# serenedb/serenedb

Measured on NVIDIA H100. Metric: filter->GROUP BY throughput (BASELINE.json configs[1]; bm25 object = configs[2]), higher is better.
Workload: dtype int64+f64

## Files before the change

### serenedb_b200/csrc/column_kernels.cuh

```cuda
#pragma once

#include "device_common.cuh"

namespace sdbg {

constexpr int kMaxPreds = 4;

struct ColDev {
  const void* values;
  const uint64_t* validity;
  int32_t type;
  int32_t pad;
};
struct PredDev {
  ColDev col;
  int32_t op;
  int32_t pad;
  int64_t lo_i, hi_i;
  double lo_f, hi_f;
};
struct PredSet {
  PredDev p[kMaxPreds];
  int32_t n;
  int32_t pad;
// ... 290 lines not shown
  GroupSlot* table;
  unsigned long long* out_of_range;
  const uint8_t* skip;
  const ForBlockDev* hdr[kMaxStreams];
  int32_t pred_stream[kMaxPreds];
  int32_t key_stream, sum_i_stream;
};
constexpr uint32_t kZoneRows = 2048;

__host__ __device__ __forceinline__ long long fkey(long long bits) { return bits ^ ((bits >> 63) & 0x7FFFFFFFFFFFFFFFll); }

__device__ __forceinline__ void fix_limbs(double w, int limb, int eunit, long long& l0, long long& l1) {
  const long long bits = __double_as_longlong(w);
  const int ex = int((bits >> 52) & 0x7FF);
  unsigned long long mant = static_cast<unsigned long long>(bits) & 0xFFFFFFFFFFFFFull;
  if (ex) mant |= 1ull << 52;
  const int s = (ex ? ex : 1) - 1075 - eunit;
  unsigned long long lo, hi = 0ull;
  if (s >= 0) { lo = mant << s; if (s) hi = mant >> (64 - s); }
  else lo = s > -64 ? mant >> (-s) : 0ull;
  l0 = static_cast<long long>(lo & ((1ull << limb) - 1ull));
  l1 = static_cast<long long>((lo >> limb) | (hi << (64 - limb)));
  if (bits < 0) { l0 = -l0; l1 = -l1; }
}
__host__ __device__ __forceinline__ double fix_total(long long s0, long long s1, int limb, int eunit) {
  long long hi = s1 >> (64 - limb);
  unsigned long long lo = static_cast<unsigned long long>(s1) << limb;
  const unsigned long long lo2 = lo + static_cast<unsigned long long>(s0);
  hi += (s0 >> 63) + (lo2 < lo ? 1 : 0);
  lo = lo2;
  const bool neg = hi < 0;
  if (neg) { lo = ~lo + 1ull; hi = ~hi + (lo == 0ull ? 1 : 0); }
  const double mag = static_cast<double>(static_cast<unsigned long long>(hi)) * 18446744073709551616.0 + static_cast<double>(lo);
  return scalbn(neg ? -mag : mag, eunit);
}

template <int kType>
__device__ __forceinline__ void load2(const unsigned char* col, uint32_t r, long long (&v)[2]) {
  if (kType == 2) {
    const int2 x = *reinterpret_cast<const int2*>(col + size_t(r) * 4u);
    v[0] = x.x; v[1] = x.y;
  } else {
    const longlong2 x = *reinterpret_cast<const longlong2*>(col + size_t(r) * 8u);
    v[0] = x.x; v[1] = x.y;
  }
}
template <int kType>
__device__ __forceinline__ uint32_t range2(const unsigned char* col, uint32_t r, long long lo, unsigned long long span) {
  long long v[2];
  load2<kType>(col, r, v);
  if (kType == 1) { v[0] = fkey(v[0]); v[1] = fkey(v[1]); }
  return (static_cast<unsigned long long>(v[0] - lo) <= span ? 1u : 0u) | (static_cast<unsigned long long>(v[1] - lo) <= span ? 2u : 0u);
}
__device__ __forceinline__ void unpack2(const unsigned char* col, uint32_t r, const uint4 h, long long (&v)[2]) {
  const unsigned long long* w = reinterpret_cast<const unsigned long long*>(col);
  const uint32_t bits = h.z;
  const long long base = static_cast<long long>((static_cast<unsigned long long>(h.y) << 32) | h.x);
  const unsigned long long mask = bits >= 64u ? ~0ull : (1ull << bits) - 1ull;
#pragma unroll
  for (int j = 0; j < 2; ++j) {
    const uint32_t bit = (r + uint32_t(j)) * bits, wi = bit >> 6, sh = bit & 63u;
    unsigned long long x = w[wi] >> sh;
    if (sh + bits > 64u) x |= w[wi + 1] << (64u - sh);
    v[j] = base + static_cast<long long>(x & mask);
  }
}
__device__ __forceinline__ uint32_t range2_for(const unsigned char* col, uint32_t r, const uint4 h, long long lo, unsigned long long span) {
  long long v[2];
  unpack2(col, r, h, v);
  return (static_cast<unsigned long long>(v[0] - lo) <= span ? 1u : 0u) | (static_cast<unsigned long long>(v[1] - lo) <= span ? 2u : 0u);
}

template <int kStages, int kTileRows, int kConsumerWarps, bool kPacked, bool kQuad, bool kFor = false>
__global__ void __launch_bounds__((kConsumerWarps + 1) * 32)
filter_groupby_tma_kernel(const TmaGroupByParams P) {
  extern __shared__ __align__(128) unsigned char smem[];
  __shared__ __align__(8) uint64_t full_bar[kStages], empty_bar[kStages];
  static_assert(!kFor || (kForGroupRows % kTileRows == 0 && kTileRows % 128 == 0), "a tile's packed slice must be 16-byte aligned");

  const uint32_t tid = threadIdx.x, warp = tid >> 5, lane = tid & 31u;
  if (tid == 0) {
    for (int s = 0; s < kStages; ++s) { mbar_init(&full_bar[s], 1u); mbar_init(&empty_bar[s], kConsumerWarps); }
    asm volatile("fence.mbarrier_init.release.cluster;" ::: "memory");
  }
  __syncthreads();
  const uint32_t stage_bytes = P.off[P.n_streams];
  const uint64_t n_tiles = (P.rows + kTileRows - 1) / kTileRows;
  uint4* const pk_hdr = reinterpret_cast<uint4*>(smem + size_t(kStages) * stage_bytes + (kQuad ? size_t(kConsumerWarps) * (2048u + 256u) : 0u));

  if (warp == kConsumerWarps) {
    if (kFor) {
      const bool mine = lane < uint32_t(P.n_streams);
      const ForBlockDev* hp = mine ? P.hdr[lane] : nullptr;
      const char* src = mine ? static_cast<const char*>(P.src[lane]) : nullptr;
      const uint32_t elem = mine ? uint32_t(P.elem[lane]) : 0u, soff = mine ? P.off[lane] : 0u;
      auto header = [&](uint64_t t) { return __ldg(reinterpret_cast<const uint4*>(hp + (t * kTileRows) / kForGroupRows)); };
      uint4 nh = make_uint4(0u, 0u, 0u, 0u);
      uint64_t nh_tile = ~0ull;
      uint32_t it = 0;
      for (uint64_t tile = blockIdx.x; tile < n_tiles; tile += gridDim.x) {
        if (P.skip != nullptr && P.skip[(tile * kTileRows) / kZoneRows]) continue;
        uint4 h = make_uint4(0u, 0u, 0u, 0u);
        if (hp != nullptr) h = nh_tile == tile ? nh : header(tile);
        const uint64_t next = tile + gridDim.x;
        if (hp != nullptr && next < n_tiles && (P.skip == nullptr || !P.skip[(next * kTileRows) / kZoneRows])) { nh = header(next); nh_tile = next; }
        const uint32_t st = it % kStages, use = it / kStages;
        ++it;
        const uint64_t row0 = tile * kTileRows;
        const uint32_t nrows = uint32_t(min(static_cast<unsigned long long>(kTileRows), static_cast<unsigned long long>(P.rows - row0)));
        uint32_t bytes = 0u;
        const char* g = nullptr;
        if (hp != nullptr) {
          bytes = (nrows * h.z + 127u) / 128u * 16u;
          g = src + uint64_t(h.w) * 8u + (row0 % kForGroupRows) * h.z / 8u;
        } else if (mine) {
          bytes = (nrows * elem + 15u) & ~15u;
          g = src + row0 * elem;
        }
        const uint32_t total = __reduce_add_sync(kFull, bytes);
        if (lane == 0) mbar_wait(&empty_bar[st], (use & 1u) ^ 1u);
        for (int s = 0; s < P.n_streams; ++s) {
          uint4 x;
          x.x = __shfl_sync(kFull, h.x, s); x.y = __shfl_sync(kFull, h.y, s); x.z = __shfl_sync(kFull, h.z, s); x.w = __shfl_sync(kFull, h.w, s);
          if (lane == 0) pk_hdr[st * kMaxStreams + s] = x;
        }
        if (lane == 0) mbar_arrive_expect_tx(&full_bar[st], total);
        __syncwarp();
        if (bytes != 0u) bulk_g2s(smem + size_t(st) * stage_bytes + soff, g, bytes, &full_bar[st]);
      }
      return;
    }
    if (lane == 0) {
      uint32_t it = 0;
      for (uint64_t tile = blockIdx.x; tile < n_tiles; tile += gridDim.x) {
        if (P.skip != nullptr && P.skip[(tile * kTileRows) / kZoneRows]) continue;
        const uint32_t st = it % kStages, use = it / kStages;
        ++it;
        mbar_wait(&empty_bar[st], (use & 1u) ^ 1u);
        const uint64_t row0 = tile * kTileRows;
        const uint32_t nrows = uint32_t(min(static_cast<unsigned long long>(kTileRows), static_cast<unsigned long long>(P.rows - row0)));
        uint32_t total = 0;
        for (int s = 0; s < P.n_streams; ++s) total += (nrows * uint32_t(P.elem[s]) + 15u) & ~15u;
        mbar_arrive_expect_tx(&full_bar[st], total);
        unsigned char* dst = smem + size_t(st) * stage_bytes;
        for (int s = 0; s < P.n_streams; ++s) {
          const uint32_t bytes = (nrows * uint32_t(P.elem[s]) + 15u) & ~15u;
          bulk_g2s(dst + P.off[s], static_cast<const char*>(P.src[s]) + row0 * uint64_t(P.elem[s]), bytes, &full_bar[st]);
        }
      }
    }
    return;
  }

  unsigned long long* const q_words = reinterpret_cast<unsigned long long*>(smem + size_t(kStages) * stage_bytes) + size_t(warp) * 256u;
  uint32_t* const q_idx = reinterpret_cast<uint32_t*>(smem + size_t(kStages) * stage_bytes + size_t(kConsumerWarps) * 2048u) + size_t(warp) * 64u;
  uint32_t it = 0;
  for (uint64_t tile = blockIdx.x; tile < n_tiles; tile += gridDim.x) {
    if (P.skip != nullptr && P.skip[(tile * kTileRows) / kZoneRows]) continue;
    const uint32_t st = it % kStages, use = it / kStages;
    ++it;
    mbar_wait(&full_bar[st], use & 1u);
    const unsigned char* base = smem + size_t(st) * stage_bytes;
    const uint64_t row0 = tile * kTileRows;
    const uint32_t nrows = uint32_t(min(static_cast<unsigned long long>(kTileRows), static_cast<unsigned long long>(P.rows - row0)));
    const uint32_t pack_word = kPacked ? uint32_t(tile % uint64_t(P.pack_tables)) : 0u;
    const uint4* const hst = pk_hdr + st * kMaxStreams;
    for (uint32_t rb = warp * 64u; rb < nrows; rb += kConsumerWarps * 64u) {
      const uint32_t r = rb + 2u * lane;
      uint32_t m = r + 1u < nrows ? 3u : r < nrows ? 1u : 0u;
#pragma unroll
      for (int i = 0; i < kMaxPreds; ++i) {
        if (i < P.n_preds) {
          const unsigned char* col = base + P.pred_off[i];
          uint32_t in;
          if (kFor && P.pred_type[i] == kTypeFor) in = range2_for(col, r, hst[P.pred_stream[i]], P.pred_lo[i], P.pred_span[i]);
          else switch (P.pred_type[i]) {
            case 0: in = range2<0>(col, r, P.pred_lo[i], P.pred_span[i]); break;
            case 1: in = range2<1>(col, r, P.pred_lo[i], P.pred_span[i]); break;
            default: in = range2<2>(col, r, P.pred_lo[i], P.pred_span[i]); break;
          }
          m &= P.pred_negate[i] ? ~in : in;
        }
      }
      if (!kQuad && m == 0u) continue;
      long long key[2], v[2] = {0, 0};
      double w[2] = {0.0, 0.0};
      if (kFor && P.key_type == kTypeFor) unpack2(base + P.key_off, r, hst[P.key_stream], key);
      else if (P.key_type == 2) load2<2>(base + P.key_off, r, key); else load2<0>(base + P.key_off, r, key);
      if (kPacked || P.has_sum_i) {
        if (kFor && P.sum_i_type == kTypeFor) unpack2(base + P.sum_i_off, r, hst[P.sum_i_stream], v);
        else if (P.sum_i_type == 2) load2<2>(base + P.sum_i_off, r, v); else load2<0>(base + P.sum_i_off, r, v);
      }
      if (P.has_sum_f) {
        const double2 x = *reinterpret_cast<const double2*>(base + P.sum_f_off + size_t(r) * 8u);
        w[0] = x.x; w[1] = x.y;
      }
      if (kQuad) {
        unsigned long long a[2][4];
        uint32_t gi[2] = {0u, 0u};
#pragma unroll
        for (int j = 0; j < 2; ++j) {
          if (!(m & (1u << j))) continue;
          const unsigned long long idx = static_cast<unsigned long long>(key[j] - P.key_min);
          if (idx >= P.key_span) { atomicAdd(P.out_of_range, 1ull); m &= ~(1u << j); continue; }
          gi[j] = uint32_t(idx);
          if (kPacked) {
            const unsigned long long pk = (1ull << P.pack_shift) + static_cast<unsigned long long>(v[j] - P.pack_bias);
            a[j][0] = pack_word == 0u ? pk : 0ull;
            a[j][1] = pack_word == 1u ? pk : 0ull;
            a[j][2] = pack_word == 2u ? pk : 0ull;
          } else {
            a[j][0] = 1ull;
            a[j][1] = !P.has_sum_i ? 0ull : P.wide_int ? (static_cast<unsigned long long>(v[j]) & 0xFFFFFFFFull) : static_cast<unsigned long long>(v[j]);
            a[j][2] = P.has_sum_i && P.wide_int ? static_cast<unsigned long long>(v[j] >> 32) : 0ull;
          }
          a[j][3] = 0ull;
          if (P.fix_limb) {
            long long l0, l1;
// ... 249 lines not shown
      case 1: static_cast<long long*>(out)[i] = static_cast<long long>(h % 1000000ull); break;
      case 2: static_cast<double*>(out)[i] = static_cast<double>(h >> 11) * 0x1.0p-53; break;
      case 3: static_cast<long long*>(out)[i] = static_cast<long long>(h % 2001ull) - 1000ll; break;
      case 4: static_cast<double*>(out)[i] = static_cast<double>(h >> 11) * 0x1.0p-53 * 1000.0; break;
      case 6: static_cast<int*>(out)[i] = static_cast<int>(h % 1000000ull); break;
      case 7: static_cast<long long*>(out)[i] = static_cast<long long>((row0 + i) / 100ull); break;
      default: static_cast<long long*>(out)[i] = static_cast<long long>(h); break;
    }
  }
}

template <typename T>
__global__ void __launch_bounds__(256)
gather_rows_kernel(const T* __restrict__ values, const unsigned long long* __restrict__ validity, const uint32_t* __restrict__ docs,
                   uint64_t n, uint64_t rows, T* __restrict__ out, unsigned char* __restrict__ out_valid) {
  for (uint64_t i = uint64_t(blockIdx.x) * blockDim.x + threadIdx.x; i < n; i += uint64_t(gridDim.x) * blockDim.x) {
    const uint64_t r = uint64_t(docs[i]) - 1ull;
    const bool inside = r < rows;
    const bool ok = inside && (validity == nullptr || ((validity[r >> 6] >> (r & 63ull)) & 1ull));
    out[i] = ok ? values[r] : T(0);
    if (out_valid != nullptr) out_valid[i] = ok ? 1u : 0u;
  }
}

__device__ __forceinline__ long long for_value(const ForBlockDev& h, const unsigned long long* w, uint32_t i) {
  unsigned long long v = 0ull;
  if (h.bits != 0u) {
    const unsigned long long mask = h.bits >= 64u ? ~0ull : ((1ull << h.bits) - 1ull);
    const uint64_t bit = uint64_t(i) * h.bits;
    const uint32_t sh = uint32_t(bit & 63ull);
    const unsigned long long lo = w[bit >> 6] >> sh;
    const unsigned long long hi = (sh != 0u && sh + h.bits > 64u) ? (w[(bit >> 6) + 1ull] << (64u - sh)) : 0ull;
    v = (lo | hi) & mask;
  }
  return h.base + static_cast<long long>(v);
}

__global__ void __launch_bounds__(256)
for_unpack_kernel(const ForBlockDev* __restrict__ headers, const unsigned long long* __restrict__ words, uint64_t rows,
                  long long* __restrict__ out) {
  const uint64_t n_groups = (rows + kForGroupRows - 1) / kForGroupRows;
  const uint32_t lane = threadIdx.x & 31u;
  for (uint64_t g = (uint64_t(blockIdx.x) * blockDim.x + threadIdx.x) >> 5; g < n_groups; g += (uint64_t(gridDim.x) * blockDim.x) >> 5) {
    const ForBlockDev h = headers[g];
    const uint64_t row0 = g * kForGroupRows;
    const uint32_t n = (rows - row0 < kForGroupRows) ? uint32_t(rows - row0) : kForGroupRows;
    for (uint32_t i = lane; i < n; i += 32u) out[row0 + i] = for_value(h, words + h.off8, i);
  }
}

__global__ void __launch_bounds__(256)
for_stats_kernel(const long long* __restrict__ values, const ForBlockDev* __restrict__ packed_hdr,
                 const unsigned long long* __restrict__ words, uint64_t rows, long long* __restrict__ zone,
                 ForBlockDev* __restrict__ hdr, unsigned long long* __restrict__ n_words) {
  const uint64_t n_groups = (rows + kForGroupRows - 1) / kForGroupRows;
  const uint32_t lane = threadIdx.x & 31u;
  for (uint64_t g = (uint64_t(blockIdx.x) * blockDim.x + threadIdx.x) >> 5; g < n_groups; g += (uint64_t(gridDim.x) * blockDim.x) >> 5) {
    const uint64_t row0 = g * kForGroupRows;
    const uint32_t n = (rows - row0 < kForGroupRows) ? uint32_t(rows - row0) : kForGroupRows;
    long long mn = 0x7FFFFFFFFFFFFFFFll, mx = -0x7FFFFFFFFFFFFFFFll - 1;
    for (uint32_t i = lane; i < n; i += 32u) {
      const long long v = words ? for_value(packed_hdr[g], words + packed_hdr[g].off8, i) : values[row0 + i];
      mn = min(mn, v); mx = max(mx, v);
    }
#pragma unroll
    for (int o = 16; o > 0; o >>= 1) { mn = min(mn, __shfl_xor_sync(kFull, mn, o)); mx = max(mx, __shfl_xor_sync(kFull, mx, o)); }
    if (lane == 0) {
      zone[2 * g] = mn; zone[2 * g + 1] = mx;
      if (!words) {
        const unsigned long long span = static_cast<unsigned long long>(mx) - static_cast<unsigned long long>(mn);
        const uint32_t bits = span == 0ull ? 0u : uint32_t(64 - __clzll(static_cast<long long>(span)));
        ForBlockDev h; h.base = mn; h.bits = bits; h.off8 = 0u;
        hdr[g] = h;
        n_words[g] = (uint64_t(n) * bits + 63u) / 64u;
      }
    }
  }
}

__global__ void __launch_bounds__(256)
for_pack_kernel(const long long* __restrict__ values, const ForBlockDev* __restrict__ stats_hdr,
                const unsigned long long* __restrict__ offsets, uint64_t rows, ForBlockDev* __restrict__ hdr,
                unsigned long long* __restrict__ words) {
  const uint64_t n_groups = (rows + kForGroupRows - 1) / kForGroupRows;
  const uint32_t lane = threadIdx.x & 31u;
  for (uint64_t g = (uint64_t(blockIdx.x) * blockDim.x + threadIdx.x) >> 5; g < n_groups; g += (uint64_t(gridDim.x) * blockDim.x) >> 5) {
    ForBlockDev h = stats_hdr[g];
    h.off8 = uint32_t(offsets[g]);
    const uint64_t row0 = g * kForGroupRows;
    const uint32_t n = (rows - row0 < kForGroupRows) ? uint32_t(rows - row0) : kForGroupRows;
    if (lane == 0) hdr[g] = h;
    const uint32_t nw = uint32_t(offsets[g + 1] - offsets[g]);
    for (uint32_t wi = lane; wi < nw; wi += 32u) {
      const uint64_t b0 = uint64_t(wi) * 64u;
      const uint32_t i0 = uint32_t(b0 / h.bits), i1 = min(n - 1u, uint32_t((b0 + 63u) / h.bits));
      unsigned long long word = 0ull;
      for (uint32_t i = i0; i <= i1; ++i) {
        const unsigned long long d = static_cast<unsigned long long>(values[row0 + i]) - static_cast<unsigned long long>(h.base);
        const uint64_t p = uint64_t(i) * h.bits;
        word |= p >= b0 ? d << (p - b0) : d >> (b0 - p);
      }
      words[h.off8 + wi] = word;
    }
    if (g + 1 == n_groups && lane == 0) words[offsets[n_groups]] = 0ull;
  }
}

}
```

### serenedb_b200/csrc/sdbg_abi.cu

```cuda
#include <cuda_runtime.h>
#include <cub/device/device_radix_sort.cuh>
#include <cub/device/device_scan.cuh>
#include <dlfcn.h>
#include <nccl.h>

#include <algorithm>
#include <array>
#include <atomic>
#include <cfloat>
#include <cmath>
#include <cstdio>
#include <cstdlib>
#include <cstring>
#include <map>
#include <memory>
#include <string>
#include <limits>
#include <thread>
#include <vector>

#include "../../include/sdbg.h"
#include "bm25_kernels.cuh"
#include "bm25_stream.cuh"
#include "bm25_merge.cuh"
#include "bm25_count.cuh"
#include "bm25_sort.cuh"
#include "column_kernels.cuh"
#include "posting_format.hpp"

using namespace sdbg;

namespace {

struct DevBuf {
  void* p = nullptr;
  size_t cap = 0;
};

struct ColumnObj {
  void* d_values = nullptr;
  void* d_packed = nullptr;
  size_t packed_bytes = 0;
  uint64_t* d_validity = nullptr;
  int type = 0;
  uint64_t rows = 0;
  bool owned = true;
  bool has_minmax = false;
  int64_t mn = 0, mx = 0;
  long long* d_zone = nullptr;
  bool zone_ok = false;
  bool has_absmax = false;
  uint64_t absmax_bits = 0;
};

}

struct sdbg_ctx {
  int device = 0;
  int sm_count = 132;
  cudaStream_t stream = nullptr;
  cudaStream_t stream2 = nullptr;
  cudaEvent_t ev_fork = nullptr, ev_join = nullptr;
  cudaEvent_t ev0 = nullptr, ev1 = nullptr;
  std::string err;
  uint64_t launches = 0;
  DevBuf scratch[16];
  DevBuf pass[4];
  DevBuf stage_raw;
  void* h_pinned = nullptr;
  size_t h_pinned_cap = 0;
  void* flush = nullptr;
  size_t flush_bytes = 0;
  cudaEvent_t ev_copy[16] = {};
  bool topk_attr_set = false;
  void* nccl_comm = nullptr;
  unsigned long long* h_oor = nullptr;
  void* h_result = nullptr;
  void* d_result = nullptr;
  unsigned long long result_seq = 0;
  size_t h_result_cap = 0;
  bool counter_zeroed = false;
  bool oor_pending = false;
  bool fix_over_pending = false;
  uint64_t zone_blocks_total = 0;
  unsigned long long* d_zone_skipped = nullptr;
  int dist_rank = 0, dist_world = 1;
  int wand = 1;
  bool profiling = false;
  struct ProfSpan { int id; cudaEvent_t a, b; };
  std::vector<ProfSpan> spans;
  std::vector<cudaEvent_t> event_pool;
};

struct sdbg_segment {
  sdbg_ctx* ctx = nullptr;
// ... 356 lines not shown
  CU(c, cudaMalloc(&s->d_norms, rows * width + 16));
  CU(c, cudaMemcpyAsync(s->d_norms, src, rows * width, cudaMemcpyHostToDevice, c->stream));
  CU(c, cudaStreamSynchronize(c->stream));
  s->norm_width = width;
  s->wand_avg_dl = nonzero ? float(double(sum) / double(nonzero)) : 0.f;
  return SDBG_OK;
}

namespace {
size_t type_width(int t) { return t == SDBG_I32 ? 4 : 8; }

uint64_t for_groups(uint64_t rows) { return (rows + kForGroupRows - 1) / kForGroupRows; }
size_t for_hdr_bytes(uint64_t rows) { return (for_groups(rows) * sizeof(ForBlockDev) + 255) & ~size_t(255); }
const ForBlockDev* for_headers(const ColumnObj& col) { return static_cast<const ForBlockDev*>(col.d_packed); }
const unsigned long long* for_words(const ColumnObj& col) {
  return reinterpret_cast<const unsigned long long*>(static_cast<const char*>(col.d_packed) + for_hdr_bytes(col.rows));
}
unsigned grid_per_group_warp(sdbg_ctx* c, uint64_t n_groups) {
  return unsigned(std::max<uint64_t>(1, std::min<uint64_t>((n_groups * 32 + 255) / 256, uint64_t(c->sm_count) * 16)));
}
int ensure_zone(sdbg_ctx* c, ColumnObj& col) {
  if (!col.d_zone) CU(c, cudaMalloc(reinterpret_cast<void**>(&col.d_zone), for_groups(col.rows) * 16));
  return SDBG_OK;
}

int raw_values(sdbg_ctx* c, ColumnObj& col, void** out) {
  if (!col.d_values && col.d_packed) {
    CU(c, cudaMalloc(&col.d_values, col.rows * 8 + 64));
    CU(c, cudaMemsetAsync(static_cast<char*>(col.d_values) + col.rows * 8, 0, 64, c->stream));
    for_unpack_kernel<<<grid_per_group_warp(c, for_groups(col.rows)), 256, 0, c->stream>>>(for_headers(col), for_words(col), col.rows,
                                                                                           static_cast<long long*>(col.d_values));
    ++c->launches;
    CU(c, cudaGetLastError());
  }
  *out = col.d_values;
  return SDBG_OK;
}

int pack_column(sdbg_ctx* c, ColumnObj& col) {
  const uint64_t rows = col.rows, n_groups = for_groups(rows);
  int rc;
  auto keep_raw = [&]() -> int {
    if (col.d_packed) { cudaFree(col.d_packed); col.d_packed = nullptr; col.packed_bytes = 0; }
    CU(c, cudaMalloc(&col.d_values, rows * 8 + 64));
    CU(c, cudaMemcpyAsync(col.d_values, c->stage_raw.p, rows * 8 + 64, cudaMemcpyDeviceToDevice, c->stream));
    return SDBG_OK;
  };
  if (rows >= (1ull << 32)) return keep_raw();
  if ((rc = ensure_zone(c, col))) return rc;
  const size_t h_bytes = (n_groups * sizeof(ForBlockDev) + 255) & ~size_t(255), n_bytes = ((n_groups + 1) * 8 + 255) & ~size_t(255);
  size_t scan_bytes = 0;
  CU(c, cub::DeviceScan::ExclusiveSum(nullptr, scan_bytes, static_cast<const unsigned long long*>(nullptr),
                                      static_cast<unsigned long long*>(nullptr), int(n_groups + 1), c->stream));
  if ((rc = ensure(c, c->scratch[12], h_bytes + 2 * n_bytes + scan_bytes))) return rc;
  char* base = static_cast<char*>(c->scratch[12].p);
  auto* s_hdr = reinterpret_cast<ForBlockDev*>(base);
  auto* s_nw = reinterpret_cast<unsigned long long*>(base + h_bytes);
  auto* s_off = reinterpret_cast<unsigned long long*>(base + h_bytes + n_bytes);
  CU(c, cudaMemsetAsync(s_nw + n_groups, 0, 8, c->stream));
  const auto* raw = static_cast<const long long*>(c->stage_raw.p);
  const unsigned grid = grid_per_group_warp(c, n_groups);
  for_stats_kernel<<<grid, 256, 0, c->stream>>>(raw, nullptr, nullptr, rows, col.d_zone, s_hdr, s_nw);
  col.zone_ok = true;
  ++c->launches;
  CU(c, cudaGetLastError());
  CU(c, cub::DeviceScan::ExclusiveSum(base + h_bytes + 2 * n_bytes, scan_bytes, s_nw, s_off, int(n_groups + 1), c->stream));
  unsigned long long total = 0;
  CU(c, cudaMemcpyAsync(&total, s_off + n_groups, 8, cudaMemcpyDeviceToHost, c->stream));
  CU(c, cudaStreamSynchronize(c->stream));
  const size_t packed_bytes = for_hdr_bytes(rows) + (total + 1) * 8 + 64;
  if (packed_bytes >= rows * 8) return keep_raw();
  if (col.d_packed && col.packed_bytes != packed_bytes) { cudaFree(col.d_packed); col.d_packed = nullptr; }
  if (!col.d_packed) CU(c, cudaMalloc(&col.d_packed, packed_bytes));
  col.packed_bytes = packed_bytes;
  CU(c, cudaMemsetAsync(static_cast<char*>(col.d_packed) + packed_bytes - 64, 0, 64, c->stream));
  for_pack_kernel<<<grid, 256, 0, c->stream>>>(raw, s_hdr, s_off, rows, static_cast<ForBlockDev*>(col.d_packed),
                                               const_cast<unsigned long long*>(for_words(col)));
  ++c->launches;
  CU(c, cudaGetLastError());
  return SDBG_OK;
}

void reset_for_packing(ColumnObj& col, uint64_t rows) {
  void* keep = nullptr;
  long long* zone = nullptr;
  size_t keep_bytes = 0;
  if (col.owned && col.rows == rows) {
    keep = col.d_packed; keep_bytes = col.packed_bytes; zone = col.d_zone;
    col.d_packed = nullptr; col.d_zone = nullptr;
  }
  free_column(col);
  col = ColumnObj{};
  col.type = SDBG_I64; col.rows = rows; col.owned = true;
  col.d_packed = keep; col.packed_bytes = keep_bytes; col.d_zone = zone;
}
}

extern "C" int sdbg_stage_column(sdbg_segment* s, uint64_t field, sdbg_type t, const void* values,
                                 const uint64_t* validity, uint64_t rows) {
  if (!s || !values || t < 0 || t > 2) return SDBG_EINVAL;
  sdbg_ctx* c = s->ctx;
  CU(c, cudaSetDevice(c->device));
  ColumnObj& col = s->cols[field];
  const size_t bytes = rows * type_width(t);
  if (t == SDBG_I64 && !validity && rows) {
    int rc;
    if ((rc = ensure(c, c->stage_raw, bytes + 64))) return rc;
    reset_for_packing(col, rows);
    CU(c, cudaMemsetAsync(static_cast<char*>(c->stage_raw.p) + bytes, 0, 64, c->stream));
    CU(c, cudaMemcpyAsync(c->stage_raw.p, values, bytes, cudaMemcpyHostToDevice, c->stream));
    return pack_column(c, col);
  }
  if (col.d_packed || !(col.owned && col.d_values && col.rows == rows && col.type == t)) {
    free_column(col);
    col = ColumnObj{};
    CU(c, cudaMalloc(&col.d_values, bytes + 64));
    CU(c, cudaMemsetAsync(static_cast<char*>(col.d_values) + bytes, 0, 64, c->stream));
  }
  col.zone_ok = false;
  col.type = t; col.rows = rows; col.owned = true; col.has_minmax = false; col.has_absmax = false;
  CU(c, cudaMemcpyAsync(col.d_values, values, bytes, cudaMemcpyHostToDevice, c->stream));
  if (validity) {
    const size_t vb = ((rows + 63) / 64) * 8;
    if (!col.d_validity) CU(c, cudaMalloc(reinterpret_cast<void**>(&col.d_validity), vb + 16));
    CU(c, cudaMemcpyAsync(col.d_validity, validity, vb, cudaMemcpyHostToDevice, c->stream));
  } else if (col.d_validity) {
    cudaFree(col.d_validity); col.d_validity = nullptr;
// ... 13 lines not shown
      const uint64_t r0 = g * kForGroupRows, r1 = std::min<uint64_t>(rows, r0 + kForGroupRows);
      int64_t mn = values[r0], mx = values[r0];
      for (uint64_t r = r0 + 1; r < r1; ++r) { mn = std::min(mn, values[r]); mx = std::max(mx, values[r]); }
      const uint64_t span = uint64_t(mx) - uint64_t(mn);
      headers[g].base = mn;
      headers[g].bits = span == 0 ? 0u : uint32_t(64 - __builtin_clzll(span));
    }
  };
  {
    std::vector<std::thread> pool;
    for (size_t t = 0; t < n_thr; ++t) pool.emplace_back(stats, n_groups * t / n_thr, n_groups * (t + 1) / n_thr);
    for (auto& th : pool) th.join();
  }
  uint64_t off = 0;
  for (uint64_t g = 0; g < n_groups; ++g) {
    const uint64_t n = std::min<uint64_t>(kForGroupRows, rows - g * kForGroupRows);
    if (off > 0xFFFFFFFFull) return SDBG_EUNSUPPORTED;
    headers[g].off8 = uint32_t(off);
    off += (n * headers[g].bits + 63) / 64;
  }
  *n_words = off + 1;
  if (*n_words > cap_words) return SDBG_ECAPACITY;
  auto pack = [&](uint64_t g0, uint64_t g1) {
    for (uint64_t g = g0; g < g1; ++g) {
      const uint32_t bits = headers[g].bits;
      if (!bits) continue;
      const uint64_t r0 = g * kForGroupRows, n = std::min<uint64_t>(kForGroupRows, rows - r0);
      uint64_t* w = words + headers[g].off8;
      const uint64_t nw = (n * bits + 63) / 64;
      std::fill(w, w + nw, 0ull);
      const uint64_t base = uint64_t(headers[g].base);
      for (uint64_t i = 0; i < n; ++i) {
        const uint64_t v = uint64_t(values[r0 + i]) - base, bit = i * bits;
        w[bit >> 6] |= v << (bit & 63);
        if ((bit & 63) + bits > 64) w[(bit >> 6) + 1] |= v >> (64 - (bit & 63));
      }
    }
  };
  {
    std::vector<std::thread> pool;
    for (size_t t = 0; t < n_thr; ++t) pool.emplace_back(pack, n_groups * t / n_thr, n_groups * (t + 1) / n_thr);
    for (auto& th : pool) th.join();
  }
  words[off] = 0;
  return SDBG_OK;
}

extern "C" int sdbg_stage_column_for(sdbg_segment* s, uint64_t field, const sdbg_for_block* headers, const uint64_t* words,
                                     uint64_t n_words, uint64_t rows) {
  if (!s || !headers || !words || !rows || !n_words) return SDBG_EINVAL;
  sdbg_ctx* c = s->ctx;
  CU(c, cudaSetDevice(c->device));
  const uint64_t n_groups = (rows + kForGroupRows - 1) / kForGroupRows;
  for (uint64_t g = 0; g < n_groups; ++g) {
    const uint64_t n = std::min<uint64_t>(kForGroupRows, rows - g * kForGroupRows);
    if (headers[g].bits > 64u || uint64_t(headers[g].off8) + (n * headers[g].bits + 63) / 64 + 1 > n_words)
      return fail(c, SDBG_EFORMAT, "bit-packed column: group outside the word stream");
  }
  ColumnObj& col = s->cols[field];
  const size_t bytes = rows * 8;
  bool aligned = rows < (1ull << 32);
  for (uint64_t g = 0; g < n_groups && aligned; ++g) aligned = (headers[g].off8 & 1u) == 0u;
  const size_t packed_bytes = for_hdr_bytes(rows) + n_words * 8 + 64;
  if (aligned && packed_bytes < bytes) {
    if (!(col.d_packed && col.packed_bytes == packed_bytes && col.rows == rows && !col.d_values && col.d_zone)) {
      free_column(col);
      col = ColumnObj{};
      col.rows = rows; col.packed_bytes = packed_bytes;
      CU(c, cudaMalloc(&col.d_packed, packed_bytes));
    }
    col.type = SDBG_I64; col.rows = rows; col.owned = true; col.has_minmax = false; col.has_absmax = false;
    CU(c, cudaMemcpyAsync(col.d_packed, headers, n_groups * sizeof(ForBlockDev), cudaMemcpyHostToDevice, c->stream));
    CU(c, cudaMemcpyAsync(const_cast<unsigned long long*>(for_words(col)), words, n_words * 8, cudaMemcpyHostToDevice, c->stream));
    CU(c, cudaMemsetAsync(static_cast<char*>(col.d_packed) + packed_bytes - 64, 0, 64, c->stream));
    { int rc = ensure_zone(c, col); if (rc) return rc; }
    col.zone_ok = true;
    for_stats_kernel<<<grid_per_group_warp(c, n_groups), 256, 0, c->stream>>>(nullptr, for_headers(col), for_words(col), rows, col.d_zone,
                                                                              nullptr, nullptr);
    ++c->launches;
    CU(c, cudaGetLastError());
    return SDBG_OK;
  }
  if (col.d_packed || !(col.owned && col.d_values && col.rows == rows && col.type == SDBG_I64)) {
    free_column(col);
    col = ColumnObj{};
    CU(c, cudaMalloc(&col.d_values, bytes + 64));
    CU(c, cudaMemsetAsync(static_cast<char*>(col.d_values) + bytes, 0, 64, c->stream));
  }
  if (col.d_validity) { cudaFree(col.d_validity); col.d_validity = nullptr; }
  col.type = SDBG_I64; col.rows = rows; col.owned = true; col.has_minmax = false; col.has_absmax = false;
  col.zone_ok = false;
  DevBuf& buf = c->scratch[12];
  const size_t hdr_bytes = (n_groups * sizeof(ForBlockDev) + 255) & ~size_t(255);
  int rc = ensure(c, buf, hdr_bytes + n_words * 8);
  if (rc) return rc;
  char* base = static_cast<char*>(buf.p);
  CU(c, cudaMemcpyAsync(base, headers, n_groups * sizeof(ForBlockDev), cudaMemcpyHostToDevice, c->stream));
  CU(c, cudaMemcpyAsync(base + hdr_bytes, words, n_words * 8, cudaMemcpyHostToDevice, c->stream));
  const unsigned grid = unsigned(std::min<uint64_t>((n_groups * 32 + 255) / 256, uint64_t(c->sm_count) * 16));
  for_unpack_kernel<<<std::max(grid, 1u), 256, 0, c->stream>>>(reinterpret_cast<const ForBlockDev*>(base),
                                                               reinterpret_cast<const unsigned long long*>(base + hdr_bytes), rows,
                                                               static_cast<long long*>(col.d_values));
  ++c->launches;
  CU(c, cudaGetLastError());
  return SDBG_OK;
}

extern "C" int sdbg_stage_column_device(sdbg_segment* s, uint64_t field, sdbg_type t, const void* d_values, uint64_t rows) {
  if (!s || !d_values || t < 0 || t > 2) return SDBG_EINVAL;
  if (rows & 1) return fail(s->ctx, SDBG_EINVAL, "borrowed device columns need an even row count (16-byte row pairs)");
  ColumnObj& col = s->cols[field];
  free_column(col);
  col = ColumnObj{};
  col.d_values = const_cast<void*>(d_values); col.type = t; col.rows = rows; col.owned = false;
  return SDBG_OK;
}

extern "C" int sdbg_column_device_ptr(sdbg_segment* s, uint64_t field, void** d_values, uint64_t* rows) {
  if (!s) return SDBG_EINVAL;
  auto it = s->cols.find(field);
  if (it == s->cols.end()) return fail(s->ctx, SDBG_ENOTFOUND, "unknown column");
  CU(s->ctx, cudaSetDevice(s->ctx->device));
  ColumnObj& col = it->second;
  void* p = nullptr;
  const int rc = raw_values(s->ctx, col, &p);
  if (rc) return rc;
  if (col.d_packed) {
    CU(s->ctx, cudaStreamSynchronize(s->ctx->stream));
    cudaFree(col.d_packed);
    col.d_packed = nullptr; col.packed_bytes = 0;
  }
// ... 2446 lines not shown
  if (avg_f64_field != UINT64_MAX && all_tma && !plan.wide_int && total_rows && absmax_bits < 0x7FF0000000000000ull &&
      env_int("SDBG_GROUPBY_FIXED", 1)) {
    int row_bits = 1;
    while ((1ull << row_bits) <= total_rows) ++row_bits;
    plan.fix_limb = std::min(37, 63 - row_bits);
    double mx; std::memcpy(&mx, &absmax_bits, 8);
    int e = 0;
    if (mx > 0) std::frexp(mx, &e);
    plan.fix_eunit = std::max(e - 2 * plan.fix_limb, -1074);
  }
  plan.quad = all_tma && (avg_f64_field == UINT64_MAX || plan.fix_limb) && env_int("SDBG_GROUPBY_QUAD", 0);
  if (!plan.quad) plan.fix_limb = 0, plan.fix_eunit = 0;
  const int shape = env_int("SDBG_GROUPBY_TMA_SHAPE", 0);
  for (size_t si = 0; si < n_segs; ++si) {
    sdbg_segment* s = segs[si];
    auto nullable = [&](uint64_t f) { auto it = s->cols.find(f); return it != s->cols.end() && it->second.d_validity != nullptr; };
    bool packed_ok = env_int("SDBG_GROUPBY_TMA", 1) != 0 && shape == 0 && !nullable(key_field) &&
                     (sum_int_field == UINT64_MAX || !nullable(sum_int_field)) && (avg_f64_field == UINT64_MAX || !nullable(avg_f64_field));
    for (size_t i = 0; i < n_preds; ++i) packed_ok = packed_ok && preds[i].op < 7 && !nullable(preds[i].field);
    GroupByParams P;
    std::memset(&P, 0, sizeof P);
    uint64_t rows = 0;
    if ((rc = pred_set(s, preds, n_preds, &P.ps, &rows, packed_ok))) return rc;
    uint64_t r = 0;
    if ((rc = col_view(s, key_field, &P.key, &r, packed_ok))) return rc;
    if (!rows) rows = r;
    if (r != rows) return fail(c, SDBG_EINVAL, "key column length differs");
    if (sum_int_field != UINT64_MAX) {
      if ((rc = col_view(s, sum_int_field, &P.sum_i, &r, packed_ok))) return rc;
      if (r != rows) return fail(c, SDBG_EINVAL, "sum_int column length differs");
      if (P.sum_i.type == SDBG_F64) return fail(c, SDBG_EINVAL, "sum_int_field is a float column");
      P.has_sum_i = 1;
    }
    if (avg_f64_field != UINT64_MAX) {
      if ((rc = col_view(s, avg_f64_field, &P.sum_f, &r))) return rc;
      if (r != rows) return fail(c, SDBG_EINVAL, "avg_f64 column length differs");
      if (P.sum_f.type != SDBG_F64) return fail(c, SDBG_EINVAL, "avg_f64_field is not a float column");
      P.has_sum_f = 1;
    }
    P.wide_int = plan.wide_int; P.count_f = plan.count_f;
    P.key_min = key_min; P.key_span = span; P.rows = rows;
    P.table = table; P.cnt_f = cnt_f; P.out_of_range = oor;
    bool any_nullable = P.key.validity || (P.has_sum_i && P.sum_i.validity) || (P.has_sum_f && P.sum_f.validity);
    for (int i = 0; i < P.ps.n; ++i) any_nullable |= P.ps.p[i].col.validity != nullptr || P.ps.p[i].op >= 7;
    if (plan.pack_tables && any_nullable) return fail(c, SDBG_EINVAL, "internal: packed accumulators planned for a nullable segment");
    if (!any_nullable && env_int("SDBG_GROUPBY_TMA", 1)) {
      TmaGroupByParams T;
      std::memset(&T, 0, sizeof T);
      auto column_of = [&](const void* id) -> ColumnObj* {
        for (auto& kv : s->cols) if (kv.second.d_values == id || (id && kv.second.d_packed == id)) return &kv.second;
        return nullptr;
      };
      const void* stream_id[kMaxStreams] = {};
      auto stream_of = [&](const ColDev& col) {
        for (int i = 0; i < T.n_streams; ++i) if (stream_id[i] == col.values) return i;
        const int n = T.n_streams++;
        stream_id[n] = col.values;
        T.elem[n] = col.type == SDBG_I32 ? 4 : 8;
        if (col.type == kTypeFor) {
          T.hdr[n] = static_cast<const ForBlockDev*>(col.values);
          T.src[n] = static_cast<const char*>(col.values) + for_hdr_bytes(rows);
        } else {
          T.src[n] = col.values;
        }
        return n;
      };
      bool never = false;
      int stream_idx[kMaxPreds];
      T.n_preds = 0;
      for (int i = 0; i < P.ps.n; ++i) {
        const PredDev& pd = P.ps.p[i];
        int64_t lo, hi; int neg = 0; bool empty = false;
        if (pd.col.type == SDBG_F64) {
          double lf = -HUGE_VAL, hf = HUGE_VAL;
          const double x = pd.lo_f;
          if (std::isnan(x) || (pd.op == SDBG_OP_BETWEEN && std::isnan(pd.hi_f))) empty = true;
          switch (pd.op) {
            case SDBG_OP_LT: if (x == -HUGE_VAL) empty = true; else hf = std::nextafter(x, -HUGE_VAL); break;
            case SDBG_OP_LE: hf = x; break;
            case SDBG_OP_GT: if (x == HUGE_VAL) empty = true; else lf = std::nextafter(x, HUGE_VAL); break;
            case SDBG_OP_GE: lf = x; break;
            case SDBG_OP_EQ: lf = hf = x; break;
            case SDBG_OP_NE: lf = hf = x; neg = 1; break;
            default: lf = x; hf = pd.hi_f; break;
          }
          if (pd.op == SDBG_OP_NE && std::isnan(x)) continue;
          if (!empty && lf > hf) empty = true;
          if (!empty) {
            if (lf == 0.0) lf = -0.0;
            if (hf == 0.0) hf = 0.0;
            int64_t bl, bh; std::memcpy(&bl, &lf, 8); std::memcpy(&bh, &hf, 8);
            lo = fkey(bl); hi = fkey(bh);
          }
        } else {
          int64_t li = INT64_MIN, hi_ = INT64_MAX;
          const int64_t x = pd.lo_i;
          switch (pd.op) {
            case SDBG_OP_LT: if (x == INT64_MIN) empty = true; else hi_ = x - 1; break;
            case SDBG_OP_LE: hi_ = x; break;
            case SDBG_OP_GT: if (x == INT64_MAX) empty = true; else li = x + 1; break;
            case SDBG_OP_GE: li = x; break;
            case SDBG_OP_EQ: li = hi_ = x; break;
            case SDBG_OP_NE: li = hi_ = x; neg = 1; break;
            default: li = x; hi_ = pd.hi_i; break;
          }
          if (li > hi_) empty = true;
          lo = li; hi = hi_;
        }
        if (empty) { if (neg) continue; never = true; break; }
        const int k = T.n_preds++;
        stream_idx[k] = stream_of(pd.col);
        T.pred_type[k] = pd.col.type; T.pred_negate[k] = neg;
// ... 1 lines not shown
      }
      if (never) continue;
      T.skip = nullptr;
      if (T.n_preds && env_int("SDBG_ZONEMAP", 1) != 0) {
        ZoneVerdictParams Z;
        std::memset(&Z, 0, sizeof Z);
        Z.n_preds = T.n_preds;
        Z.n_blocks = (rows + kZoneRows - 1) / kZoneRows;
        bool any_zone = false;
        for (int k2 = 0; k2 < T.n_preds; ++k2) {
          Z.lo[k2] = T.pred_lo[k2]; Z.span[k2] = T.pred_span[k2]; Z.negate[k2] = T.pred_negate[k2];
          ColumnObj* co = column_of(stream_id[stream_idx[k2]]);
          if (!co || co->d_validity) continue;
          if (!co->zone_ok) {
            if (!co->d_zone) CU(c, cudaMalloc(reinterpret_cast<void**>(&co->d_zone), Z.n_blocks * 16));
            co->zone_ok = true;
            const unsigned zg = unsigned(std::min<uint64_t>((Z.n_blocks + 7) / 8, uint64_t(c->sm_count) * 8));
            const auto* vals = static_cast<const unsigned char*>(co->d_values);
            if (co->type == SDBG_F64) zonemap_kernel<1><<<zg, 256, 0, c->stream>>>(vals, rows, co->d_zone);
            else if (co->type == SDBG_I32) zonemap_kernel<2><<<zg, 256, 0, c->stream>>>(vals, rows, co->d_zone);
            else zonemap_kernel<0><<<zg, 256, 0, c->stream>>>(vals, rows, co->d_zone);
            ++c->launches;
          }
          Z.zone[k2] = co->d_zone;
          any_zone = true;
        }
        if (any_zone) {
          DevBuf& b_skip = c->scratch[13];
          if ((rc = ensure(c, b_skip, Z.n_blocks + 16))) return rc;
          if (!c->d_zone_skipped) CU(c, cudaMalloc(reinterpret_cast<void**>(&c->d_zone_skipped), 8));
          if (si == 0) { CU(c, cudaMemsetAsync(c->d_zone_skipped, 0, 8, c->stream)); c->zone_blocks_total = 0; }
          const unsigned vg = unsigned(std::min<uint64_t>((Z.n_blocks + 255) / 256, uint64_t(c->sm_count) * 4));
          zone_verdict_kernel<<<vg, 256, 0, c->stream>>>(Z, static_cast<uint8_t*>(b_skip.p), c->d_zone_skipped);
          ++c->launches;
          c->zone_blocks_total += Z.n_blocks;
          T.skip = static_cast<const uint8_t*>(b_skip.p);
        }
      }
      const int key_s = stream_of(P.key);
      const int sum_i_s = P.has_sum_i ? stream_of(P.sum_i) : -1;
      const int sum_f_s = P.has_sum_f ? stream_of(P.sum_f) : -1;
      T.key_type = P.key.type; T.sum_i_type = P.has_sum_i ? P.sum_i.type : 0;
      T.has_sum_i = P.has_sum_i; T.has_sum_f = P.has_sum_f;
      T.debug_skip = env_int("SDBG_GROUPBY_DEBUG", 0);
      T.wide_int = plan.wide_int; T.key_min = key_min; T.key_span = span; T.rows = rows; T.table = table; T.out_of_range = oor;
      T.pack_shift = plan.pack_shift; T.pack_tables = plan.pack_tables; T.pack_bias = plan.pack_bias;
      T.fix_limb = plan.fix_limb; T.fix_eunit = plan.fix_eunit;
      for (int i = 0; i < T.n_preds; ++i) T.pred_stream[i] = stream_idx[i];
      T.key_stream = key_s; T.sum_i_stream = sum_i_s >= 0 ? sum_i_s : 0;
      bool any_for = false;
      for (int i = 0; i < T.n_streams; ++i) any_for |= T.hdr[i] != nullptr;
      auto set_offsets = [&](int tile_rows) {
        uint32_t o = 0;
        for (int i = 0; i < T.n_streams; ++i) { T.off[i] = o; o += uint32_t(T.elem[i]) * uint32_t(tile_rows); }
        T.off[T.n_streams] = o;
        for (int i = 0; i < T.n_preds; ++i) T.pred_off[i] = T.off[stream_idx[i]];
        T.key_off = T.off[key_s];
        T.sum_i_off = sum_i_s >= 0 ? T.off[sum_i_s] : 0;
        T.sum_f_off = sum_f_s >= 0 ? T.off[sum_f_s] : 0;
      };
      const bool quad = plan.quad != 0;
      auto launch = [&](auto kern, int stages, int tile_rows, int consumer_warps) -> int {
        set_offsets(tile_rows);
        const size_t smem = size_t(stages) * size_t(T.off[T.n_streams]) + (quad ? size_t(consumer_warps) * (2048 + 256) : 0) +
                            (any_for ? size_t(stages) * kMaxStreams * 16 : 0);
        CU(c, cudaFuncSetAttribute(kern, cudaFuncAttributeMaxDynamicSharedMemorySize, int(smem)));
        const size_t fit = std::max<size_t>(1, (220 * 1024) / (smem + 2048));
        const size_t by_threads = std::max<size_t>(1, 2048 / (size_t(consumer_warps + 1) * 32));
        int resident = 0;
        CU(c, cudaOccupancyMaxActiveBlocksPerMultiprocessor(&resident, kern, (consumer_warps + 1) * 32, smem));
        const unsigned per_sm = unsigned(std::max<size_t>(1, std::min<size_t>({fit, by_threads, size_t(env_int("SDBG_GROUPBY_TMA_CTAS", 8)), size_t(resident)})));
        const unsigned grid = unsigned(c->sm_count) * per_sm;
        ProfScope ps_(c, kProfGroupBy);
        kern<<<grid, (consumer_warps + 1) * 32, smem, c->stream>>>(T);
        return SDBG_OK;
      };
      int lrc;
      switch (shape) {
        case 1: lrc = launch(filter_groupby_tma_kernel<4, 256, 8, false, false>, 4, 256, 8); break;
        case 2: lrc = launch(filter_groupby_tma_kernel<4, 512, 16, false, false>, 4, 512, 16); break;
        case 3: lrc = launch(filter_groupby_tma_kernel<3, 256, 8, false, false>, 3, 256, 8); break;
        case 4: lrc = launch(filter_groupby_tma_kernel<4, 1024, 16, false, false>, 4, 1024, 16); break;
        default: {
#define SDBG_GB_LAUNCH(ST, FOR) \
          (plan.pack_tables ? (quad ? launch(filter_groupby_tma_kernel<ST, kGroupByTileRows, 8, true, true, FOR>, ST, kGroupByTileRows, 8) \
                                    : launch(filter_groupby_tma_kernel<ST, kGroupByTileRows, 8, true, false, FOR>, ST, kGroupByTileRows, 8)) \
                            : (quad ? launch(filter_groupby_tma_kernel<ST, kGroupByTileRows, 8, false, true, FOR>, ST, kGroupByTileRows, 8) \
                                    : launch(filter_groupby_tma_kernel<ST, kGroupByTileRows, 8, false, false, FOR>, ST, kGroupByTileRows, 8)))
          const int stages = env_int("SDBG_GROUPBY_TMA_STAGES", kGroupByDefaultStages);
          if (any_for) lrc = stages == 2 ? SDBG_GB_LAUNCH(2, true) : stages == 3 ? SDBG_GB_LAUNCH(3, true) : SDBG_GB_LAUNCH(4, true);
          else lrc = stages == 2 ? SDBG_GB_LAUNCH(2, false) : stages == 3 ? SDBG_GB_LAUNCH(3, false) : SDBG_GB_LAUNCH(4, false);
#undef SDBG_GB_LAUNCH
          break;
        }
      }
      if (lrc) return lrc;
    } else {
      const unsigned grid = unsigned(c->sm_count) * unsigned(env_int("SDBG_GROUPBY_CTAS_PER_SM", 8));
      ProfScope ps_(c, kProfGroupBy);
      filter_groupby_kernel<2><<<grid, 256, 0, c->stream>>>(P);
    }
    ++c->launches;
    CU(c, cudaGetLastError());
  }
  groupby_pack_kernel<<<c->sm_count * 2, 256, 0, c->stream>>>(table, plan.count_f ? cnt_f : nullptr, span,
                                                               static_cast<long long*>(d_i64), static_cast<double*>(d_f64),
                                                               plan.pack_shift, plan.pack_tables, plan.pack_bias, plan.fix_limb, plan.fix_eunit);
  ++c->launches;
  CU(c, cudaGetLastError());
  if (defer_check) {
    if (!c->h_oor) CU(c, cudaHostAlloc(reinterpret_cast<void**>(&c->h_oor), 16, cudaHostAllocDefault));
    CU(c, cudaMemcpyAsync(c->h_oor, oor, 8, cudaMemcpyDeviceToHost, c->stream));
    c->oor_pending = true;
  } else {
    unsigned long long h_oor = 0;
    CU(c, cudaMemcpyAsync(&h_oor, oor, 8, cudaMemcpyDeviceToHost, c->stream));
    CU(c, cudaStreamSynchronize(c->stream));
    if (h_oor) return fail(c, SDBG_EINVAL, "GROUP BY key outside [key_min, key_min + span)");
// ... 463 lines not shown
```

Before: 79220.

## Size FOR stream smem slots by max bit width and use 32-bit unpack

```diff
diff --git a/serenedb_b200/csrc/column_kernels.cuh b/serenedb_b200/csrc/column_kernels.cuh
--- a/serenedb_b200/csrc/column_kernels.cuh
+++ b/serenedb_b200/csrc/column_kernels.cuh
@@ -366,10 +366,26 @@
   if (kType == 1) { v[0] = fkey(v[0]); v[1] = fkey(v[1]); }
   return (static_cast<unsigned long long>(v[0] - lo) <= span ? 1u : 0u) | (static_cast<unsigned long long>(v[1] - lo) <= span ? 2u : 0u);
 }
+__device__ __forceinline__ void unpack2_narrow(const unsigned char* col, uint32_t r, uint32_t bits, uint32_t (&x)[2]) {
+  const uint32_t* w = reinterpret_cast<const uint32_t*>(col);
+  const uint32_t mask = bits >= 32u ? ~0u : (1u << bits) - 1u;
+#pragma unroll
+  for (int j = 0; j < 2; ++j) {
+    const uint32_t bit = (r + uint32_t(j)) * bits, wi = bit >> 5;
+    x[j] = __funnelshift_r(w[wi], w[wi + 1], bit & 31u) & mask;
+  }
+}
 __device__ __forceinline__ void unpack2(const unsigned char* col, uint32_t r, const uint4 h, long long (&v)[2]) {
-  const unsigned long long* w = reinterpret_cast<const unsigned long long*>(col);
   const uint32_t bits = h.z;
   const long long base = static_cast<long long>((static_cast<unsigned long long>(h.y) << 32) | h.x);
+  if (bits <= 32u) {
+    uint32_t x[2];
+    unpack2_narrow(col, r, bits, x);
+    v[0] = base + static_cast<long long>(x[0]);
+    v[1] = base + static_cast<long long>(x[1]);
+    return;
+  }
+  const unsigned long long* w = reinterpret_cast<const unsigned long long*>(col);
   const unsigned long long mask = bits >= 64u ? ~0ull : (1ull << bits) - 1ull;
 #pragma unroll
   for (int j = 0; j < 2; ++j) {
@@ -380,6 +396,18 @@
   }
 }
 __device__ __forceinline__ uint32_t range2_for(const unsigned char* col, uint32_t r, const uint4 h, long long lo, unsigned long long span) {
+  if (h.z <= 32u) {
+    const unsigned long long base = (static_cast<unsigned long long>(h.y) << 32) | h.x, top = (1ull << h.z) - 1ull;
+    const unsigned long long ulo = static_cast<unsigned long long>(lo), uhi = ulo + span;
+    if (static_cast<long long>(uhi) < static_cast<long long>(base)) return 0u;
+    const unsigned long long tlo = lo <= static_cast<long long>(base) ? 0ull : ulo - base;
+    if (tlo > top) return 0u;
+    const unsigned long long thi = min(uhi - base, top);
+    uint32_t x[2];
+    unpack2_narrow(col, r, h.z, x);
+    const uint32_t l32 = uint32_t(tlo), s32 = uint32_t(thi - tlo);
+    return (x[0] - l32 <= s32 ? 1u : 0u) | (x[1] - l32 <= s32 ? 2u : 0u);
+  }
   long long v[2];
   unpack2(col, r, h, v);
   return (static_cast<unsigned long long>(v[0] - lo) <= span ? 1u : 0u) | (static_cast<unsigned long long>(v[1] - lo) <= span ? 2u : 0u);
@@ -401,6 +429,7 @@
   const uint32_t stage_bytes = P.off[P.n_streams];
   const uint64_t n_tiles = (P.rows + kTileRows - 1) / kTileRows;
   uint4* const pk_hdr = reinterpret_cast<uint4*>(smem + size_t(kStages) * stage_bytes + (kQuad ? size_t(kConsumerWarps) * (2048u + 256u) : 0u));
+  uint2* const pk_desc = reinterpret_cast<uint2*>(pk_hdr + kStages * kMaxStreams);
 
   if (warp == kConsumerWarps) {
     if (kFor) {
@@ -412,7 +441,9 @@
       uint4 nh = make_uint4(0u, 0u, 0u, 0u);
       uint64_t nh_tile = ~0ull;
       uint32_t it = 0;
-      for (uint64_t tile = blockIdx.x; tile < n_tiles; tile += gridDim.x) {
+      const uint32_t n_words = kPacked ? uint32_t(P.pack_tables) : 1u, pw_step = gridDim.x % n_words;
+      uint32_t pw = blockIdx.x % n_words;
+      for (uint64_t tile = blockIdx.x; tile < n_tiles; tile += gridDim.x, pw = pw + pw_step >= n_words ? pw + pw_step - n_words : pw + pw_step) {
         if (P.skip != nullptr && P.skip[(tile * kTileRows) / kZoneRows]) continue;
         uint4 h = make_uint4(0u, 0u, 0u, 0u);
         if (hp != nullptr) h = nh_tile == tile ? nh : header(tile);
@@ -433,14 +464,21 @@
         }
         const uint32_t total = __reduce_add_sync(kFull, bytes);
         if (lane == 0) mbar_wait(&empty_bar[st], (use & 1u) ^ 1u);
-        for (int s = 0; s < P.n_streams; ++s) {
-          uint4 x;
-          x.x = __shfl_sync(kFull, h.x, s); x.y = __shfl_sync(kFull, h.y, s); x.z = __shfl_sync(kFull, h.z, s); x.w = __shfl_sync(kFull, h.w, s);
-          if (lane == 0) pk_hdr[st * kMaxStreams + s] = x;
+        __syncwarp();
+        if (mine) pk_hdr[st * kMaxStreams + lane] = h;
+        __syncwarp();
+        if (lane == 0) {
+          pk_desc[st] = make_uint2(nrows, pw);
+          mbar_arrive_expect_tx(&full_bar[st], total);
         }
-        if (lane == 0) mbar_arrive_expect_tx(&full_bar[st], total);
         __syncwarp();
         if (bytes != 0u) bulk_g2s(smem + size_t(st) * stage_bytes + soff, g, bytes, &full_bar[st]);
+      }
+      if (lane == 0) {
+        const uint32_t st = it % kStages, use = it / kStages;
+        mbar_wait(&empty_bar[st], (use & 1u) ^ 1u);
+        pk_desc[st] = make_uint2(0u, 0u);
+        mbar_arrive(&full_bar[st]);
       }
       return;
     }
@@ -469,15 +507,26 @@
   unsigned long long* const q_words = reinterpret_cast<unsigned long long*>(smem + size_t(kStages) * stage_bytes) + size_t(warp) * 256u;
   uint32_t* const q_idx = reinterpret_cast<uint32_t*>(smem + size_t(kStages) * stage_bytes + size_t(kConsumerWarps) * 2048u) + size_t(warp) * 64u;
   uint32_t it = 0;
-  for (uint64_t tile = blockIdx.x; tile < n_tiles; tile += gridDim.x) {
-    if (P.skip != nullptr && P.skip[(tile * kTileRows) / kZoneRows]) continue;
-    const uint32_t st = it % kStages, use = it / kStages;
-    ++it;
-    mbar_wait(&full_bar[st], use & 1u);
+  for (uint64_t tile = blockIdx.x;; tile += gridDim.x) {
+    uint32_t st, nrows, pack_word;
+    if (kFor) {
+      st = it % kStages;
+      mbar_wait(&full_bar[st], (it / kStages) & 1u);
+      ++it;
+      const uint2 d = pk_desc[st];
+      if (d.x == 0u) break;
+      nrows = d.x; pack_word = d.y;
+    } else {
+      if (tile >= n_tiles) break;
+      if (P.skip != nullptr && P.skip[(tile * kTileRows) / kZoneRows]) continue;
+      st = it % kStages;
+      mbar_wait(&full_bar[st], (it / kStages) & 1u);
+      ++it;
+      const uint64_t row0 = tile * kTileRows;
+      nrows = uint32_t(min(static_cast<unsigned long long>(kTileRows), static_cast<unsigned long long>(P.rows - row0)));
+      pack_word = kPacked ? uint32_t(tile % uint64_t(P.pack_tables)) : 0u;
+    }
     const unsigned char* base = smem + size_t(st) * stage_bytes;
-    const uint64_t row0 = tile * kTileRows;
-    const uint32_t nrows = uint32_t(min(static_cast<unsigned long long>(kTileRows), static_cast<unsigned long long>(P.rows - row0)));
-    const uint32_t pack_word = kPacked ? uint32_t(tile % uint64_t(P.pack_tables)) : 0u;
     const uint4* const hst = pk_hdr + st * kMaxStreams;
     for (uint32_t rb = warp * 64u; rb < nrows; rb += kConsumerWarps * 64u) {
       const uint32_t r = rb + 2u * lane;
@@ -833,7 +882,7 @@
 __global__ void __launch_bounds__(256)
 for_stats_kernel(const long long* __restrict__ values, const ForBlockDev* __restrict__ packed_hdr,
                  const unsigned long long* __restrict__ words, uint64_t rows, long long* __restrict__ zone,
-                 ForBlockDev* __restrict__ hdr, unsigned long long* __restrict__ n_words) {
+                 ForBlockDev* __restrict__ hdr, unsigned long long* __restrict__ n_words, unsigned int* __restrict__ max_bits) {
   const uint64_t n_groups = (rows + kForGroupRows - 1) / kForGroupRows;
   const uint32_t lane = threadIdx.x & 31u;
   for (uint64_t g = (uint64_t(blockIdx.x) * blockDim.x + threadIdx.x) >> 5; g < n_groups; g += (uint64_t(gridDim.x) * blockDim.x) >> 5) {
@@ -854,6 +903,7 @@
         ForBlockDev h; h.base = mn; h.bits = bits; h.off8 = 0u;
         hdr[g] = h;
         n_words[g] = (uint64_t(n) * bits + 63u) / 64u;
+        atomicMax(max_bits, bits);
       }
     }
   }
diff --git a/serenedb_b200/csrc/sdbg_abi.cu b/serenedb_b200/csrc/sdbg_abi.cu
--- a/serenedb_b200/csrc/sdbg_abi.cu
+++ b/serenedb_b200/csrc/sdbg_abi.cu
@@ -41,6 +41,7 @@
   void* d_values = nullptr;
   void* d_packed = nullptr;
   size_t packed_bytes = 0;
+  uint32_t for_max_bits = 0;
   uint64_t* d_validity = nullptr;
   int type = 0;
   uint64_t rows = 0;
@@ -503,27 +504,33 @@
   size_t scan_bytes = 0;
   CU(c, cub::DeviceScan::ExclusiveSum(nullptr, scan_bytes, static_cast<const unsigned long long*>(nullptr),
                                       static_cast<unsigned long long*>(nullptr), int(n_groups + 1), c->stream));
-  if ((rc = ensure(c, c->scratch[12], h_bytes + 2 * n_bytes + scan_bytes))) return rc;
+  const size_t mb_off = h_bytes + 2 * n_bytes + ((scan_bytes + 15) & ~size_t(15));
+  if ((rc = ensure(c, c->scratch[12], mb_off + 16))) return rc;
   char* base = static_cast<char*>(c->scratch[12].p);
   auto* s_hdr = reinterpret_cast<ForBlockDev*>(base);
   auto* s_nw = reinterpret_cast<unsigned long long*>(base + h_bytes);
   auto* s_off = reinterpret_cast<unsigned long long*>(base + h_bytes + n_bytes);
+  auto* s_max_bits = reinterpret_cast<unsigned int*>(base + mb_off);
   CU(c, cudaMemsetAsync(s_nw + n_groups, 0, 8, c->stream));
+  CU(c, cudaMemsetAsync(s_max_bits, 0, 4, c->stream));
   const auto* raw = static_cast<const long long*>(c->stage_raw.p);
   const unsigned grid = grid_per_group_warp(c, n_groups);
-  for_stats_kernel<<<grid, 256, 0, c->stream>>>(raw, nullptr, nullptr, rows, col.d_zone, s_hdr, s_nw);
+  for_stats_kernel<<<grid, 256, 0, c->stream>>>(raw, nullptr, nullptr, rows, col.d_zone, s_hdr, s_nw, s_max_bits);
   col.zone_ok = true;
   ++c->launches;
   CU(c, cudaGetLastError());
   CU(c, cub::DeviceScan::ExclusiveSum(base + h_bytes + 2 * n_bytes, scan_bytes, s_nw, s_off, int(n_groups + 1), c->stream));
   unsigned long long total = 0;
+  unsigned int max_bits = 0;
   CU(c, cudaMemcpyAsync(&total, s_off + n_groups, 8, cudaMemcpyDeviceToHost, c->stream));
+  CU(c, cudaMemcpyAsync(&max_bits, s_max_bits, 4, cudaMemcpyDeviceToHost, c->stream));
   CU(c, cudaStreamSynchronize(c->stream));
   const size_t packed_bytes = for_hdr_bytes(rows) + (total + 1) * 8 + 64;
   if (packed_bytes >= rows * 8) return keep_raw();
   if (col.d_packed && col.packed_bytes != packed_bytes) { cudaFree(col.d_packed); col.d_packed = nullptr; }
   if (!col.d_packed) CU(c, cudaMalloc(&col.d_packed, packed_bytes));
   col.packed_bytes = packed_bytes;
+  col.for_max_bits = max_bits;
   CU(c, cudaMemsetAsync(static_cast<char*>(col.d_packed) + packed_bytes - 64, 0, 64, c->stream));
   for_pack_kernel<<<grid, 256, 0, c->stream>>>(raw, s_hdr, s_off, rows, static_cast<ForBlockDev*>(col.d_packed),
                                                const_cast<unsigned long long*>(for_words(col)));
@@ -643,8 +650,10 @@
   sdbg_ctx* c = s->ctx;
   CU(c, cudaSetDevice(c->device));
   const uint64_t n_groups = (rows + kForGroupRows - 1) / kForGroupRows;
+  uint32_t max_bits = 0;
   for (uint64_t g = 0; g < n_groups; ++g) {
     const uint64_t n = std::min<uint64_t>(kForGroupRows, rows - g * kForGroupRows);
+    max_bits = std::max(max_bits, headers[g].bits);
     if (headers[g].bits > 64u || uint64_t(headers[g].off8) + (n * headers[g].bits + 63) / 64 + 1 > n_words)
       return fail(c, SDBG_EFORMAT, "bit-packed column: group outside the word stream");
   }
@@ -661,13 +670,14 @@
       CU(c, cudaMalloc(&col.d_packed, packed_bytes));
     }
     col.type = SDBG_I64; col.rows = rows; col.owned = true; col.has_minmax = false; col.has_absmax = false;
+    col.for_max_bits = max_bits;
     CU(c, cudaMemcpyAsync(col.d_packed, headers, n_groups * sizeof(ForBlockDev), cudaMemcpyHostToDevice, c->stream));
     CU(c, cudaMemcpyAsync(const_cast<unsigned long long*>(for_words(col)), words, n_words * 8, cudaMemcpyHostToDevice, c->stream));
     CU(c, cudaMemsetAsync(static_cast<char*>(col.d_packed) + packed_bytes - 64, 0, 64, c->stream));
     { int rc = ensure_zone(c, col); if (rc) return rc; }
     col.zone_ok = true;
     for_stats_kernel<<<grid_per_group_warp(c, n_groups), 256, 0, c->stream>>>(nullptr, for_headers(col), for_words(col), rows, col.d_zone,
-                                                                              nullptr, nullptr);
+                                                                              nullptr, nullptr, nullptr);
     ++c->launches;
     CU(c, cudaGetLastError());
     return SDBG_OK;
@@ -3220,12 +3230,15 @@
         return nullptr;
       };
       const void* stream_id[kMaxStreams] = {};
+      uint32_t slot_bits[kMaxStreams] = {};
       auto stream_of = [&](const ColDev& col) {
         for (int i = 0; i < T.n_streams; ++i) if (stream_id[i] == col.values) return i;
         const int n = T.n_streams++;
         stream_id[n] = col.values;
         T.elem[n] = col.type == SDBG_I32 ? 4 : 8;
+        slot_bits[n] = uint32_t(T.elem[n]) * 8u;
         if (col.type == kTypeFor) {
+          slot_bits[n] = column_of(col.values)->for_max_bits;
           T.hdr[n] = static_cast<const ForBlockDev*>(col.values);
           T.src[n] = static_cast<const char*>(col.values) + for_hdr_bytes(rows);
         } else {
@@ -3333,7 +3346,7 @@
       for (int i = 0; i < T.n_streams; ++i) any_for |= T.hdr[i] != nullptr;
       auto set_offsets = [&](int tile_rows) {
         uint32_t o = 0;
-        for (int i = 0; i < T.n_streams; ++i) { T.off[i] = o; o += uint32_t(T.elem[i]) * uint32_t(tile_rows); }
+        for (int i = 0; i < T.n_streams; ++i) { T.off[i] = o; o += (slot_bits[i] * uint32_t(tile_rows) / 8u + 15u) & ~15u; }
         T.off[T.n_streams] = o;
         for (int i = 0; i < T.n_preds; ++i) T.pred_off[i] = T.off[stream_idx[i]];
         T.key_off = T.off[key_s];
@@ -3344,7 +3357,7 @@
       auto launch = [&](auto kern, int stages, int tile_rows, int consumer_warps) -> int {
         set_offsets(tile_rows);
         const size_t smem = size_t(stages) * size_t(T.off[T.n_streams]) + (quad ? size_t(consumer_warps) * (2048 + 256) : 0) +
-                            (any_for ? size_t(stages) * kMaxStreams * 16 : 0);
+                            (any_for ? size_t(stages) * (kMaxStreams * 16 + 8) : 0);
         CU(c, cudaFuncSetAttribute(kern, cudaFuncAttributeMaxDynamicSharedMemorySize, int(smem)));
         const size_t fit = std::max<size_t>(1, (220 * 1024) / (smem + 2048));
         const size_t by_threads = std::max<size_t>(1, 2048 / (size_t(consumer_warps + 1) * 32));
```

Result: faster. 80710, median of 6 (+1.9%).
